# MyrtleSoftware/myrtlespeech

Measured on AMD Instinct MI355X. Metric: audio-sec/s (RTF), DS2 5xBiLSTM-1024 encoder forward + CTC greedy, 80-feature 10 s clips @ batch 32/GPU, higher is better.
Workload: dtype f16x3 (f32 split in fp16 hi+lo, 3 fp16 MFMA passes, f32 acc: LSTM, projections, conv1/2, FC1; FC2/CTC/decode f32)

## Files before the change

include/ms_hotpath.h:

```cpp
#ifndef MS_HOTPATH_H
#define MS_HOTPATH_H

#include <stddef.h>
#include <stdint.h>

#ifdef __cplusplus
extern "C" {
#endif

#define MS_ABI_VERSION 4

enum {
  MS_OK = 0,
  MS_ERR_INVALID = 1,
  MS_ERR_HIP = 2,
  MS_ERR_WORKSPACE = 3,
  MS_ERR_TIMEOUT = 4,
  MS_ERR_UNSUPPORTED = 5
};

enum { MS_CELL_LSTM = 0, MS_CELL_GRU = 1, MS_CELL_RNN_TANH = 2, MS_CELL_HARD_LSTM = 3 };

enum { MS_ACT_NONE = 0, MS_ACT_CLAMP = 1  };

int ms_abi_version(void);
const char* ms_last_error(void);


int ms_mask_time_(float* x, const int32_t* lens, int N, int inner, int T, void* stream);

size_t ms_maskconv_packed_bytes(int Cout, int Cin_g, int KF, int KT, int groups);

int ms_maskconv_pack(const float* w, void* packed, int Cout, int Cin_g, int KF, int KT, int groups, void* stream);

int ms_maskconv_forward(const float* x, const int32_t* lens, const void* packed_w, const float* bias, float* y,
                        int N, int Cin, int Fin, int Tin, int Cout, int Fout, int Tout, int KF, int KT, int SF,
                        int ST, int DF, int DT, int pad_f_l, int pad_t_l, int groups, int act, float act_lo,
                        float act_hi, void* stream);

size_t ms_maskconv_cl_packed_bytes(int Cout, int Cin, int KF, int KT);
int ms_maskconv_cl_pack(const float* w, void* packed, int Cout, int Cin, int KF, int KT, void* stream);
size_t ms_maskconv_cl_workspace_bytes(int N, int Cin, int Fin, int Tin);
int ms_maskconv_cl_forward(const float* x, const int32_t* lens, const void* packed_w, const float* bias, float* y,
                           int N, int Cin, int Fin, int Tin, int Cout, int Fout, int Tout, int KF, int KT, int SF,
                           int ST, int DF, int DT, int pad_f_l, int pad_t_l, int act, float act_lo, float act_hi,
                           void* workspace, size_t workspace_bytes, void* stream);

size_t ms_maskconv_fwin_packed_bytes(int Cout, int KF, int KT);
int ms_maskconv_fwin_pack(const float* w, void* packed, int Cout, int KF, int KT, void* stream);
size_t ms_maskconv_fwin_workspace_bytes(int N, int Tin, int KF, int SF, int Fout);
int ms_maskconv_fwin_forward(const float* x, const int32_t* lens, const void* packed_w, const float* bias, float* y, int N,
                             int Fin, int Tin, int Cout, int Fout, int Tout, int KF, int KT, int SF, int ST, int DT,
                             int pad_f_l, int pad_t_l, int act, float act_lo, float act_hi, void* workspace,
                             size_t workspace_bytes, void* stream);

size_t ms_maskconv1d_gemm_packed_bytes(int Cout, int Cin, int KT);
int ms_maskconv1d_gemm_pack(const float* w, void* packed, int Cout, int Cin, int KT, void* stream);
size_t ms_maskconv1d_gemm_workspace_bytes(int N, int Cin, int Tout, int Cout, int KT);
int ms_maskconv1d_gemm_forward(const float* x, const int32_t* lens, const void* packed, const float* bias, float* y, int N,
                               int Cin, int Tin, int Cout, int Tout, int KT, int ST, int DT, int pad_l, int act,
                               float act_lo, float act_hi, void* workspace, size_t workspace_bytes, void* stream);

int ms_nct_to_tnc(const float* x, float* y, int N, int CF, int T, void* stream);

int ms_clamp(const float* x, float* y, size_t n, float lo, float hi, void* stream);


int ms_linear_forward(const float* x, const float* w, const float* bias, float* y, int M, int K, int N, int act,
                      float act_lo, float act_hi, void* stream);

#define MS_LINEAR_FEW_ROWS 1
size_t ms_linear_splitk_workspace_bytes(int M, int K, int N, int flags);
int ms_linear_splitk_forward(const float* x, const float* w, const float* bias, float* y, int M, int K, int N, int act,
                             float act_lo, float act_hi, int flags, void* workspace, size_t workspace_bytes, void* stream);

size_t ms_linear_split_workspace_bytes(int M, int K, int N);
int ms_linear_split_forward(const float* x, const float* w, const float* bias, float* y, int M, int K, int N, int act,
                            float act_lo, float act_hi, void* workspace, size_t workspace_bytes, void* stream);

size_t ms_linear_split_packed_bytes(int K, int N);
int ms_linear_split_pack(const float* w, void* packed, int K, int N, void* stream);
int ms_linear_split_forward_packed(const float* x, const void* packed_w, const float* bias, float* y, int M, int K, int N, int act,
                                   float act_lo, float act_hi, void* workspace, size_t workspace_bytes, void* stream);


int ms_lookahead_forward(const float* x, const float* w, float* y, int N, int F, int T, int ctx, long xs_n,
                         long xs_f, long xs_t, long ys_n, long ys_f, long ys_t, int act, float act_lo,
// ... 180 lines not shown
```

myrtlespeech_amd/_lib.py:

```python
import ctypes
import os
import re
from ctypes import POINTER, c_char_p, c_double, c_float, c_int, c_int32, c_long, c_size_t, c_void_p

import torch

_HERE = os.path.dirname(os.path.abspath(__file__))
LIB_PATH = os.environ.get("MS_HOTPATH_LIB") or os.path.join(_HERE, "libms_hotpath.so")
HEADER_PATH = os.path.join(os.path.dirname(_HERE), "include", "ms_hotpath.h")

MS_OK = 0
ABI_VERSION = 4
ERR_NAMES = {1: "MS_ERR_INVALID", 2: "MS_ERR_HIP", 3: "MS_ERR_WORKSPACE", 4: "MS_ERR_TIMEOUT", 5: "MS_ERR_UNSUPPORTED"}

CELL_LSTM, CELL_GRU, CELL_RNN_TANH, CELL_HARD_LSTM = 0, 1, 2, 3
ACT_NONE, ACT_CLAMP = 0, 1
LINEAR_FEW_ROWS = 1
PROF_KINDS = 9

_P = c_void_p
_PP = POINTER(c_void_p)

SIGNATURES = {
    "ms_abi_version": (c_int, []),
    "ms_last_error": (c_char_p, []),
    "ms_mask_time_": (c_int, [_P, _P, c_int, c_int, c_int, _P]),
    "ms_maskconv_packed_bytes": (c_size_t, [c_int, c_int, c_int, c_int, c_int]),
    "ms_maskconv_pack": (c_int, [_P, _P, c_int, c_int, c_int, c_int, c_int, _P]),
    "ms_maskconv_forward": (c_int, [_P, _P, _P, _P, _P] + [c_int] * 17 + [c_float, c_float, _P]),
    "ms_maskconv_cl_packed_bytes": (c_size_t, [c_int, c_int, c_int, c_int]),
    "ms_maskconv_cl_pack": (c_int, [_P, _P, c_int, c_int, c_int, c_int, _P]),
    "ms_maskconv_cl_workspace_bytes": (c_size_t, [c_int, c_int, c_int, c_int]),
    "ms_maskconv_cl_forward": (c_int, [_P, _P, _P, _P, _P] + [c_int] * 16 + [c_float, c_float, _P, c_size_t, _P]),
    "ms_maskconv_fwin_packed_bytes": (c_size_t, [c_int, c_int, c_int]),
    "ms_maskconv_fwin_pack": (c_int, [_P, _P, c_int, c_int, c_int, _P]),
    "ms_maskconv_fwin_workspace_bytes": (c_size_t, [c_int, c_int, c_int, c_int, c_int]),
    "ms_maskconv_fwin_forward": (c_int, [_P, _P, _P, _P, _P] + [c_int] * 14 + [c_float, c_float, _P, c_size_t, _P]),
    "ms_maskconv1d_gemm_packed_bytes": (c_size_t, [c_int, c_int, c_int]),
    "ms_maskconv1d_gemm_pack": (c_int, [_P, _P, c_int, c_int, c_int, _P]),
    "ms_maskconv1d_gemm_workspace_bytes": (c_size_t, [c_int] * 5),
    "ms_maskconv1d_gemm_forward": (c_int, [_P, _P, _P, _P, _P] + [c_int] * 10 + [c_float, c_float, _P, c_size_t, _P]),
    "ms_nct_to_tnc": (c_int, [_P, _P, c_int, c_int, c_int, _P]),
    "ms_clamp": (c_int, [_P, _P, c_size_t, c_float, c_float, _P]),
    "ms_linear_forward": (c_int, [_P, _P, _P, _P, c_int, c_int, c_int, c_int, c_float, c_float, _P]),
    "ms_linear_splitk_workspace_bytes": (c_size_t, [c_int, c_int, c_int, c_int]),
    "ms_linear_splitk_forward": (c_int, [_P, _P, _P, _P, c_int, c_int, c_int, c_int, c_float, c_float, c_int, _P, c_size_t, _P]),
    "ms_linear_split_workspace_bytes": (c_size_t, [c_int, c_int, c_int]),
    "ms_linear_split_forward": (c_int, [_P, _P, _P, _P, c_int, c_int, c_int, c_int, c_float, c_float, _P, c_size_t, _P]),
    "ms_linear_split_packed_bytes": (c_size_t, [c_int, c_int]),
    "ms_linear_split_pack": (c_int, [_P, _P, c_int, c_int, _P]),
    "ms_linear_split_forward_packed": (c_int, [_P, _P, _P, _P, c_int, c_int, c_int, c_int, c_float, c_float, _P, c_size_t, _P]),
    "ms_lookahead_forward": (c_int, [_P, _P, _P, c_int, c_int, c_int, c_int] + [c_long] * 6 + [c_int, c_float, c_float, _P]),
    "ms_lookahead_window_forward": (c_int, [_P, _P, _P, c_int, c_int, c_int, c_int, c_int] + [c_long] * 6 + [c_int, c_float, c_float, _P]),
    "ms_rnn_packed_bytes": (c_size_t, [c_int, c_int, c_int, c_int]),
    "ms_ctc_status": (c_int, [_P, _P]),
    "ms_rnn_padded_hidden": (c_int, [c_int, c_int, c_int]),
    "ms_rnn_hx_preinit": (c_int, [c_int] * 8 + [_P, c_size_t, _P]),
    "ms_rnn_pack": (c_int, [c_int, c_int, c_int, c_int, _PP, _PP, _PP, _PP, _P, _P]),
    "ms_rnn_workspace_bytes": (c_size_t, [c_int] * 6),
    "ms_rnn_layer_forward": (c_int, [c_int, _P, _P, _P, c_int, _P, _P, _P, _P, _P] + [c_int] * 5 + [_P, c_size_t, _P]),
    "ms_rnn_layer_forward_ex": (c_int, [c_int, _P, _P, _P, c_int, _P, _P, _P, _P, _P] + [c_int] * 6 + [_P, c_size_t, _P]),
    "ms_rnn_layer_chains_planes": (c_int, [c_int, c_int, c_int]),
    "ms_rnn_layer_is_wide": (c_int, [c_int] * 4),
    "ms_rnn_stack_overlap_ok": (c_int, [c_int] * 7),
    "ms_rnn_stack_forward": (c_int, [c_int, _P, _P, _P, c_int, _P, _P, _P, _P, _P] + [c_int] * 7 + [_P, c_size_t, _P]),
    "ms_rnn_status": (c_int, [_P, _P]),
    "ms_rnn_debug_offset": (c_size_t, [c_int] * 6),
    "ms_rnn_layer_packs_rows": (c_int, [c_int] * 6),
    "ms_gemm_set_variant": (c_int, [c_int]),
    "ms_prof_enable": (c_int, [c_int]),
# ... 248 lines not shown
```

myrtlespeech_amd/csrc/conv_cl.hip:

```cpp
#include <algorithm>
#include <type_traits>

#include "common.h"

namespace {

typedef unsigned u32x4 __attribute__((ext_vector_type(4)));
typedef unsigned u32x2 __attribute__((ext_vector_type(2)));
typedef __bf16 bf16x8 __attribute__((ext_vector_type(8)));
typedef _Float16 f16x8 __attribute__((ext_vector_type(8)));

constexpr int CL_F = 2;

struct ClP {
  int N, Cin, Fin, Tin, Cout, Fout, Tout, KF, KT, SF, ST, DF, DT, pad_f, pad_t;
  int KG;
  int PW;
  int co_tiles;
  int act;
  float lo, hi;
  int FP;
};

__device__ __forceinline__ unsigned bf16b(float x) { return (unsigned)__builtin_bit_cast(unsigned short, (__bf16)x); }
// ... 120 lines not shown
            } else {
              const u32x4 bl = *reinterpret_cast<const u32x4*>(Pl + poff);
              acc[f] = ms::mfma_32x32x16<HM>(ah, bh, acc[f]);
              acc[f] = ms::mfma_32x32x16<HM>(al, bh, acc[f]);
              acc[f] = ms::mfma_32x32x16<HM>(ah, bl, acc[f]);
            }
          }
        }
      }
    }
    __syncthreads();
  }

  const int t = t0 + wt * 32 + l31;
  const float winv = scale_word[1];
  if (t < p.Tout) {
#pragma unroll
    for (int f = 0; f < CL_F; ++f) {
      const int fo = fo0 + wf * CL_F + f;
      if (fo >= p.Fout) continue;
#pragma unroll
      for (int r = 0; r < 16; ++r) {
        const int co = tile * 32 + ms::mfma32_row(r, lane);
        if (co < p.Cout) {
          float v = acc[f][r] * winv + (bias ? bias[co] : 0.f);
          if (p.act == MS_ACT_CLAMP) v = fminf(fmaxf(v, p.lo), p.hi);
          y[(((size_t)n * p.Cout + co) * p.Fout + fo) * p.Tout + t] = v;
        }
      }
    }
  }
}


constexpr int SH_RB = 12;
constexpr int SH_KT = 11;

template <int P>
__global__ __launch_bounds__(256, 1) void maskconv_cl_short_kernel(const unsigned short* __restrict__ xh,
                                                                   const unsigned short* __restrict__ xl,
                                                                   const int32_t* __restrict__ lens,
                                                                   const unsigned short* __restrict__ wp,
                                                                   const float* __restrict__ bias, float* __restrict__ y, ClP p,
                                                                   int RB, int RIN, const float* __restrict__ scale_word) {
  constexpr bool F16 = ms::prec_one_plane(P), HM = P == ms::PREC_F16X3;
  const float winv = scale_word[1];
  extern __shared__ __attribute__((aligned(16))) char lds[];
  const int tid = threadIdx.x, lane = tid & 63, wave = __builtin_amdgcn_readfirstlane(tid >> 6);
  const int c16 = lane & 15, q = lane >> 4;
  const int fo0 = blockIdx.x * RB, cb = blockIdx.y, n = blockIdx.z;
  const int PW = p.PW;
  const int row_bytes = PW * 64;
  char* Ph = lds;
  char* Pl = lds + (size_t)RIN * row_bytes;
  const int len = lens ? min(lens[n], p.Tin) : p.Tin;
  const int fin_lo = fo0 * p.SF - p.pad_f;

  for (int i = tid; i < RIN * PW * 4; i += 256) {
    const int kg = i & 3, rq = i >> 2;
    const int r = rq / PW, fq = rq - r * PW;
    const int fin = fin_lo + r, tin = fq - p.pad_t;
    u32x4 vh = {0u, 0u, 0u, 0u}, vl = {0u, 0u, 0u, 0u};
    if (fin >= 0 && fin < p.Fin && tin >= 0 && tin < len) {
      const size_t off = (((size_t)n * p.Fin + fin) * p.Tin + tin) * 32 + kg * 8;
      vh = *reinterpret_cast<const u32x4*>(xh + off);
      if (!F16) vl = *reinterpret_cast<const u32x4*>(xl + off);
// ... 173 lines not shown
  }
  return 0;
}

template <bool WIN>
int conv_cl_launch(const ClP& p, int wf, size_t lds, const unsigned short* xh, const unsigned short* xl, const int32_t* lens,
                   const void* packed_w, const float* bias, float* y, hipStream_t stream, const float* scale_word) {
  static ms::DeviceOnce attr_once;
  if (attr_once.need()) {
#define MS_CL_ATTR(PP)                                                                                                                     \
    MS_HIP(hipFuncSetAttribute((const void*)maskconv_cl_kernel<PP, WIN, 1>, hipFuncAttributeMaxDynamicSharedMemorySize, 160 * 1024));   \
    MS_HIP(hipFuncSetAttribute((const void*)maskconv_cl_kernel<PP, WIN, 4>, hipFuncAttributeMaxDynamicSharedMemorySize, 160 * 1024));
    MS_CL_ATTR(ms::PREC_BF16X3) MS_CL_ATTR(ms::PREC_F16) MS_CL_ATTR(ms::PREC_F16X3)
#undef MS_CL_ATTR
    attr_once.done();
  }
  const int prec = ms::split_mode();
  const int tt = 128 / wf, rf = CL_F * wf;
  dim3 grid(ms::cdiv(p.Tout, tt), ms::cdiv(p.Fout, rf), p.N * p.co_tiles);
  const unsigned short* wq = (const unsigned short*)packed_w;
#define MS_CL_LAUNCH(WF_)                                                                                                             \
  if (prec == ms::PREC_F16) hipLaunchKernelGGL((maskconv_cl_kernel<ms::PREC_F16, WIN, WF_>), grid, dim3(256), lds, stream, xh, xl, lens, wq, bias, y, p, scale_word); \
  else if (prec == ms::PREC_F16X3) hipLaunchKernelGGL((maskconv_cl_kernel<ms::PREC_F16X3, WIN, WF_>), grid, dim3(256), lds, stream, xh, xl, lens, wq, bias, y, p, scale_word); \
  else hipLaunchKernelGGL((maskconv_cl_kernel<ms::PREC_BF16X3, WIN, WF_>), grid, dim3(256), lds, stream, xh, xl, lens, wq, bias, y, p, scale_word);
  if (wf == 4) { MS_CL_LAUNCH(4) } else { MS_CL_LAUNCH(1) }
#undef MS_CL_LAUNCH
  MS_LAUNCH_CHECK();
  return MS_OK;
}

inline int fwin_kfp(int KF) { return ms::cdiv(KF, 16) * 16; }
inline int fwin_fp(int KF, int SF, int Fout) { return ms::cdiv((Fout - 1) * SF + fwin_kfp(KF), 32) * 32; }

}

static size_t fwin_plane_bytes(int Cout, int KF, int KT) {
  return ms::align_up((size_t)2 * KT * (fwin_kfp(KF) / 8) * (ms::cdiv(Cout, 32) * 32) * 8 * sizeof(unsigned short), 256);
}
extern "C" size_t ms_maskconv_fwin_packed_bytes(int Cout, int KF, int KT) {
  if (Cout <= 0 || KF <= 0 || KT <= 0) return 0;
  return fwin_plane_bytes(Cout, KF, KT) + 256;
}

extern "C" int ms_maskconv_fwin_pack(const float* w, void* packed, int Cout, int KF, int KT, void* stream) {
  MS_REQUIRE(w && packed, "null pointer");
  MS_REQUIRE(Cout > 0 && KF > 0 && KT > 0, "bad shape");
  const int cout_pad = ms::cdiv(Cout, 32) * 32, KG = fwin_kfp(KF) / 8;
  const size_t plane = (size_t)KT * KG * cout_pad * 8;
  const int blocks = (int)std::min<size_t>((plane + 255) / 256, 2048);
  float* scale_word = (float*)((char*)packed + fwin_plane_bytes(Cout, KF, KT));
  const int rc = ms::weight_scale_launch(w, (size_t)Cout * KF * KT, scale_word, ms::split_mode(), (hipStream_t)stream);
  if (rc != MS_OK) return rc;
  hipLaunchKernelGGL(conv_fwin_pack_kernel, dim3(blocks), dim3(256), 0, (hipStream_t)stream, w, (unsigned short*)packed, Cout,
                     KF, KT, KG, cout_pad, ms::split_mode(), scale_word);
  MS_LAUNCH_CHECK();
  return MS_OK;
}

extern "C" size_t ms_maskconv_fwin_workspace_bytes(int N, int Tin, int KF, int SF, int Fout) {
  if (N <= 0 || Tin <= 0 || KF <= 0 || SF <= 0 || Fout <= 0) return 0;
  return ms::align_up((size_t)N * Tin * fwin_fp(KF, SF, Fout) * 4, 256);
}

extern "C" int ms_maskconv_fwin_forward(const float* x, const int32_t* lens, const void* packed_w, const float* bias, float* y,
                                        int N, int Fin, int Tin, int Cout, int Fout, int Tout, int KF, int KT, int SF, int ST,
                                        int DT, int pad_f_l, int pad_t_l, int act, float act_lo, float act_hi, void* workspace,
                                        size_t workspace_bytes, void* stream_) {
  ms::ProfScope prof_span(MS_PROF_CONV, (hipStream_t)stream_);
  MS_REQUIRE(x && packed_w && y && workspace, "null pointer");
  MS_REQUIRE(N > 0 && Fin > 0 && Tin > 0 && Cout > 0 && Fout > 0 && Tout > 0, "bad shape");
  MS_REQUIRE(KF > 0 && KT > 0 && SF > 0 && ST > 0 && DT > 0 && pad_f_l >= 0 && pad_t_l >= 0, "bad kernel");
  MS_REQUIRE(SF % 2 == 0, "feature stride must be even (4-byte aligned window loads)");
  MS_REQUIRE(act == MS_ACT_NONE || act == MS_ACT_CLAMP, "bad act");
  if (workspace_bytes < ms_maskconv_fwin_workspace_bytes(N, Tin, KF, SF, Fout)) {
    ms::set_error("ms_maskconv_fwin_forward: workspace too small");
    return MS_ERR_WORKSPACE;
  }
  hipStream_t stream = (hipStream_t)stream_;
  ClP p;
  p.N = N; p.Cin = fwin_kfp(KF); p.Fin = 1; p.Tin = Tin; p.Cout = Cout; p.Fout = Fout; p.Tout = Tout; p.KF = 1; p.KT = KT;
  p.SF = SF; p.ST = ST; p.DF = 1; p.DT = DT; p.pad_f = 0; p.pad_t = pad_t_l; p.KG = p.Cin / 8;
  p.co_tiles = ms::cdiv(Cout, 32);
  p.act = act; p.lo = act_lo; p.hi = act_hi;
  p.FP = fwin_fp(KF, SF, Fout);
  size_t lds = 0;
  const int wf = conv_cl_plan(p, &lds);
  if (wf == 0 || (size_t)N * Tin * p.FP * 2 >= ((size_t)1 << 31)) {
    ms::set_error("ms_maskconv_fwin_forward: shape outside the LDS / grid budget");
    return MS_ERR_UNSUPPORTED;
  }
  unsigned short* xh = (unsigned short*)workspace;
  unsigned short* xl = xh + (size_t)N * Tin * p.FP;
  const int prec = ms::split_mode();
  const bool f16 = prec == ms::PREC_F16;
  hipLaunchKernelGGL(ft_to_tf_split_kernel, dim3(ms::cdiv(Tin, 32), ms::cdiv(p.FP, 32), N), dim3(32, 8), 0, stream, x, xh, xl,
                     Fin, Tin, p.FP, pad_f_l, prec);
  MS_LAUNCH_CHECK();
  return conv_cl_launch<true>(p, wf, lds, xh, xl, lens, packed_w, bias, y, stream,
                              (const float*)((const char*)packed_w + fwin_plane_bytes(Cout, KF, KT)));
}

static size_t cl_plane_bytes(int Cout, int Cin, int KF, int KT) {
  return ms::align_up((size_t)2 * KF * KT * (Cin / 8) * (ms::cdiv(Cout, 32) * 32) * 8 * sizeof(unsigned short), 256);
}
extern "C" size_t ms_maskconv_cl_packed_bytes(int Cout, int Cin, int KF, int KT) {
  if (Cout <= 0 || Cin <= 0 || Cin % 16 || KF <= 0 || KT <= 0) return 0;
  return cl_plane_bytes(Cout, Cin, KF, KT) + 256;
}

extern "C" int ms_maskconv_cl_pack(const float* w, void* packed, int Cout, int Cin, int KF, int KT, void* stream) {
  MS_REQUIRE(w && packed, "null pointer");
  MS_REQUIRE(Cout > 0 && Cin > 0 && Cin % 16 == 0 && KF > 0 && KT > 0, "bad shape (Cin must be a multiple of 16)");
  const int cout_pad = ms::cdiv(Cout, 32) * 32;
  const size_t plane = (size_t)KF * KT * (Cin / 8) * cout_pad * 8;
  const int blocks = (int)std::min<size_t>((plane + 255) / 256, 2048);
  float* scale_word = (float*)((char*)packed + cl_plane_bytes(Cout, Cin, KF, KT));
  const int rc = ms::weight_scale_launch(w, (size_t)Cout * Cin * KF * KT, scale_word, ms::split_mode(), (hipStream_t)stream);
  if (rc != MS_OK) return rc;
  hipLaunchKernelGGL(conv_cl_pack_kernel, dim3(blocks), dim3(256), 0, (hipStream_t)stream, w, (unsigned short*)packed, Cout,
                     Cin, KF, KT, cout_pad, ms::split_mode(), scale_word);
  MS_LAUNCH_CHECK();
  return MS_OK;
}

extern "C" size_t ms_maskconv_cl_workspace_bytes(int N, int Cin, int Fin, int Tin) {
  if (N <= 0 || Cin <= 0 || Fin <= 0 || Tin <= 0) return 0;
  return ms::align_up((size_t)N * Cin * Fin * Tin * 4, 256);
}

extern "C" int ms_maskconv_cl_forward(const float* x, const int32_t* lens, const void* packed_w, const float* bias, float* y,
                                      int N, int Cin, int Fin, int Tin, int Cout, int Fout, int Tout, int KF, int KT,
                                      int SF, int ST, int DF, int DT, int pad_f_l, int pad_t_l, int act, float act_lo,
                                      float act_hi, void* workspace, size_t workspace_bytes, void* stream_) {
  ms::ProfScope prof_span(MS_PROF_CONV, (hipStream_t)stream_);
  MS_REQUIRE(x && packed_w && y && workspace, "null pointer");
  MS_REQUIRE(N > 0 && Cin > 0 && Cin % 16 == 0 && Fin > 0 && Tin > 0 && Cout > 0 && Fout > 0 && Tout > 0, "bad shape");
  MS_REQUIRE(KF > 0 && KT > 0 && SF > 0 && ST > 0 && DF > 0 && DT > 0 && pad_f_l >= 0 && pad_t_l >= 0, "bad kernel");
  MS_REQUIRE(act == MS_ACT_NONE || act == MS_ACT_CLAMP, "bad act");
  if (workspace_bytes < ms_maskconv_cl_workspace_bytes(N, Cin, Fin, Tin)) {
    ms::set_error("ms_maskconv_cl_forward: workspace too small");
    return MS_ERR_WORKSPACE;
  }
  hipStream_t stream = (hipStream_t)stream_;
  ClP p;
  p.N = N; p.Cin = Cin; p.Fin = Fin; p.Tin = Tin; p.Cout = Cout; p.Fout = Fout; p.Tout = Tout; p.KF = KF; p.KT = KT;
  p.SF = SF; p.ST = ST; p.DF = DF; p.DT = DT; p.pad_f = pad_f_l; p.pad_t = pad_t_l; p.KG = Cin / 8;
  p.co_tiles = ms::cdiv(Cout, 32);
  p.act = act; p.lo = act_lo; p.hi = act_hi;
  p.FP = 0;
  size_t lds = 0;
  const int wf = conv_cl_plan(p, &lds);
  if (wf == 0) {
    ms::set_error("ms_maskconv_cl_forward: shape outside the LDS / grid budget");
    return MS_ERR_UNSUPPORTED;
  }
  const float* scale_word = (const float*)((const char*)packed_w + cl_plane_bytes(Cout, Cin, KF, KT));
  unsigned short* xh = (unsigned short*)workspace;
  unsigned short* xl = xh + (size_t)N * Cin * Fin * Tin;
  MS_REQUIRE(N * Fin <= 65535, "N*Fin exceeds grid limits");
  const int prec = ms::split_mode();
  const bool f16 = prec == ms::PREC_F16;
  hipLaunchKernelGGL(nchw_to_cl_split_kernel, dim3(ms::cdiv(Tin, 32), ms::cdiv(Cin, 32), N * Fin), dim3(32, 8), 0, stream, x,
                     xh, xl, Cin, Fin, Tin, prec);
  MS_LAUNCH_CHECK();
  {
    int RB = 0, RIN = 0;
    size_t slds = 0;
    if (conv_cl_short_plan(p, f16, &RB, &RIN, &slds)) {
      static ms::DeviceOnce attr_once;
      if (attr_once.need()) {
        MS_HIP(hipFuncSetAttribute((const void*)maskconv_cl_short_kernel<ms::PREC_BF16X3>, hipFuncAttributeMaxDynamicSharedMemorySize, 160 * 1024));
        MS_HIP(hipFuncSetAttribute((const void*)maskconv_cl_short_kernel<ms::PREC_F16>, hipFuncAttributeMaxDynamicSharedMemorySize, 160 * 1024));
        MS_HIP(hipFuncSetAttribute((const void*)maskconv_cl_short_kernel<ms::PREC_F16X3>, hipFuncAttributeMaxDynamicSharedMemorySize, 160 * 1024));
        attr_once.done();
      }
      ClP ps = p;
      ps.PW = Tout + KT - 1;
      const dim3 grid(ms::cdiv(Fout, RB), ms::cdiv(Cout, 16), N);
      const unsigned short* wq = (const unsigned short*)packed_w;
      auto kern = prec == ms::PREC_F16 ? maskconv_cl_short_kernel<ms::PREC_F16>
                  : prec == ms::PREC_F16X3 ? maskconv_cl_short_kernel<ms::PREC_F16X3> : maskconv_cl_short_kernel<ms::PREC_BF16X3>;
      hipLaunchKernelGGL(kern, grid, dim3(256), slds, stream, xh, xl, lens, wq, bias, y, ps, RB, RIN, scale_word);
      MS_LAUNCH_CHECK();
      return MS_OK;
    }
  }
  return conv_cl_launch<false>(p, wf, lds, xh, xl, lens, packed_w, bias, y, stream, scale_word);
}
```

myrtlespeech_amd/model/cnn.py:

```python
from enum import Enum
import os
from typing import List, Optional, Tuple, TypeVar, Union

import torch

from myrtlespeech_amd import _lib


class PaddingMode(Enum):

    NONE = 0
    SAME = 1


def pad_same(length: int, kernel_size: int, stride: int = 1, dilation: int = 1) -> Tuple[int, int]:
    for name, v in (("length", length), ("kernel_size", kernel_size), ("stride", stride), ("dilation", dilation)):
        if v <= 0:
            raise ValueError(f"{name}={v} must be > 0")
    span = dilation * (kernel_size - 1) + 1
    n_out = (length + stride - 1) // stride
    total = stride * n_out - 1 + span - length
    left = total // 2
    return left, total - left

# ... 74 lines not shown
    n, cin, fin, tin = x4.shape
    cout, _, kf, kt = weight4.shape
    (sf, st), (df, dt) = stride, dilation
    if same:
        pt = pad_same(tin, kt, st, dt)
        pf = pad_same(fin, kf, sf, df)
    else:
        pt = pf = (0, 0)
    if time_pads is not None:
        pt = (int(time_pads[0]), int(time_pads[1]))
    fout = (fin + sum(pf) - (df * (kf - 1) + 1)) // sf + 1
    tout = (tin + sum(pt) - (dt * (kt - 1) + 1)) // st + 1
    if fout <= 0 or tout <= 0:
        raise RuntimeError("convolution output would be empty")
    host_in = _lib.host_lens(seq_lens).to(seq_lens.dtype)
    new_host = out_lens(host_in, kt, st, dt, sum(pt))
    new_lens = _lib.attach_host(_lib.upload(new_host), new_host)
    y = torch.empty((n, cout, fout, tout), dtype=torch.float32, device="cuda")
    lens_dev = _lib.lens_i32(seq_lens)
    a, lo, hi = (_lib.ACT_NONE, 0.0, 0.0) if act is None else (_lib.ACT_CLAMP, act[0], act[1])
    b = None if bias is None else _lib.f32c(bias.detach())
    big = 2.0 * y.numel() * cin * kf * kt >= float(os.environ.get("MS_CONV_MFMA_MIN_FLOPS", "1e9"))
    if _lib.split_precision() and groups == 1 and fin == 1 and kf == 1 and sf == 1 and pf == (0, 0) and cin * kt >= 64 and big:
        pk = packed.get_gemm1d(weight4)
        nbytes = lib.ms_maskconv1d_gemm_workspace_bytes(n, cin, tout, cout, kt)
        ws = packed.workspace.get(nbytes)
        _lib.check(lib.ms_maskconv1d_gemm_forward(_lib.ptr(x4), _lib.ptr(lens_dev), _lib.ptr(pk), _lib.ptr(b), _lib.ptr(y), n,
                                                  cin, tin, cout, tout, kt, st, dt, pt[0], a, lo, hi, _lib.ptr(ws), nbytes,
                                                  _lib.stream_ptr()), "ms_maskconv1d_gemm_forward")
        return y, new_lens
    if _lib.split_precision() and groups == 1 and cin % 16 == 0 and big:
        pk = packed.get_cl(weight4)
        ws = packed.workspace.get(lib.ms_maskconv_cl_workspace_bytes(n, cin, fin, tin))
        rc = lib.ms_maskconv_cl_forward(_lib.ptr(x4), _lib.ptr(lens_dev), _lib.ptr(pk), _lib.ptr(b), _lib.ptr(y), n, cin,
                                        fin, tin, cout, fout, tout, kf, kt, sf, st, df, dt, pf[0], pt[0], a, lo, hi,
                                        _lib.ptr(ws), ws.numel(), _lib.stream_ptr())
        if rc != 5:
            _lib.check(rc, "ms_maskconv_cl_forward")
            return y, new_lens
    big_fwin = 2.0 * y.numel() * cin * kf * kt >= float(os.environ.get("MS_CONV_MFMA_MIN_FLOPS", "2e8"))
    if (_lib.split_precision() and groups == 1 and cin == 1 and df == 1 and sf % 2 == 0 and kf >= 16 and big_fwin
            and os.environ.get("MS_CONV_FWIN") != "0"):
        pk = packed.get_fwin(weight4)
        nbytes = lib.ms_maskconv_fwin_workspace_bytes(n, tin, kf, sf, fout)
        ws = packed.workspace.get(nbytes)
        rc = lib.ms_maskconv_fwin_forward(_lib.ptr(x4), _lib.ptr(lens_dev), _lib.ptr(pk), _lib.ptr(b), _lib.ptr(y), n, fin,
                                          tin, cout, fout, tout, kf, kt, sf, st, dt, pf[0], pt[0], a, lo, hi, _lib.ptr(ws),
                                          nbytes, _lib.stream_ptr())
        if rc != 5:
            _lib.check(rc, "ms_maskconv_fwin_forward")
            return y, new_lens
    pk = packed.get(weight4, groups)
    _lib.check(lib.ms_maskconv_forward(_lib.ptr(x4), _lib.ptr(lens_dev), _lib.ptr(pk), _lib.ptr(b), _lib.ptr(y), n, cin,
                                       fin, tin, cout, fout, tout, kf, kt, sf, st, df, dt, pf[0], pt[0], groups, a, lo,
                                       hi, _lib.stream_ptr()), "ms_maskconv_forward")
    return y, new_lens


def _mask_in_place(acts: torch.Tensor, seq_lens: torch.Tensor):
    if acts.is_cuda and acts.dtype == torch.float32 and acts.is_contiguous():
        n, t = acts.shape[0], acts.shape[-1]
        h = _lib.host_lens(seq_lens)
        if h.numel() == n and n and int(h.min()) >= t:
            return True
        inner = acts.numel() // (n * t)
        lens_dev = _lib.lens_i32(seq_lens)
        _lib.check(_lib.load().ms_mask_time_(_lib.ptr(acts), _lib.ptr(lens_dev), n, inner, t, _lib.stream_ptr()),
                   "ms_mask_time_")
        return True
    return False


class MaskConv1d(torch.nn.Conv1d):

    def __init__(self, in_channels: int, out_channels: int, kernel_size: int, stride: int = 1,
                 padding_mode: PaddingMode = PaddingMode.NONE, dilation: int = 1, groups: int = 1, bias: bool = True):
        super().__init__(in_channels=in_channels, out_channels=out_channels, kernel_size=kernel_size, stride=stride,
                         dilation=dilation, groups=groups, bias=bias)
        if padding_mode not in (PaddingMode.NONE, PaddingMode.SAME):
            raise ValueError(f"unknown padding mode {padding_mode}")
        self._padding_mode = padding_mode
# ... 83 lines not shown
```

Before: 26910.

## Add specialized pipelined MFMA conv kernel for KT=11 channel-last and fwin convs

Adds a fixed-shape conv kernel specialized for the DS2 conv shapes (KT=11, KG=4 or 6). It stages input rows and weight taps in LDS with register prefetch of the next kf slice or tap group, double-buffers operand reads, and interleaves MFMA with LDS reads using scheduling barriers. Both the conv1 fwin path and the conv2 channel-last path try this kernel first and fall back to the generic one when the shape does not match. It adds code specialized to these exact shapes. The large LDS footprint may also limit occupancy.

```diff
diff --git a/include/ms_hotpath.h b/include/ms_hotpath.h
--- a/include/ms_hotpath.h
+++ b/include/ms_hotpath.h
@@ -53,6 +53,16 @@
                              int Fin, int Tin, int Cout, int Fout, int Tout, int KF, int KT, int SF, int ST, int DT,
                              int pad_f_l, int pad_t_l, int act, float act_lo, float act_hi, void* workspace,
                              size_t workspace_bytes, void* stream);
+
+int ms_maskconv_cl_fast_supported(int Cin, int KF, int KT, int ST, int DT, int Tout, int fwin);
+int ms_maskconv_cl_fast_forward(const float* x, const int32_t* lens, const void* packed_w, const float* bias, float* y,
+                                int N, int Cin, int Fin, int Tin, int Cout, int Fout, int Tout, int KF, int KT, int SF,
+                                int ST, int DF, int DT, int pad_f_l, int pad_t_l, int act, float act_lo, float act_hi,
+                                void* workspace, size_t workspace_bytes, void* stream);
+int ms_maskconv_fwin_fast_forward(const float* x, const int32_t* lens, const void* packed_w, const float* bias, float* y,
+                                  int N, int Fin, int Tin, int Cout, int Fout, int Tout, int KF, int KT, int SF, int ST,
+                                  int DT, int pad_f_l, int pad_t_l, int act, float act_lo, float act_hi, void* workspace,
+                                  size_t workspace_bytes, void* stream);
 
 size_t ms_maskconv1d_gemm_packed_bytes(int Cout, int Cin, int KT);
 int ms_maskconv1d_gemm_pack(const float* w, void* packed, int Cout, int Cin, int KT, void* stream);
diff --git a/myrtlespeech_amd/_lib.py b/myrtlespeech_amd/_lib.py
--- a/myrtlespeech_amd/_lib.py
+++ b/myrtlespeech_amd/_lib.py
@@ -36,6 +36,9 @@
     "ms_maskconv_fwin_pack": (c_int, [_P, _P, c_int, c_int, c_int, _P]),
     "ms_maskconv_fwin_workspace_bytes": (c_size_t, [c_int, c_int, c_int, c_int, c_int]),
     "ms_maskconv_fwin_forward": (c_int, [_P, _P, _P, _P, _P] + [c_int] * 14 + [c_float, c_float, _P, c_size_t, _P]),
+    "ms_maskconv_cl_fast_supported": (c_int, [c_int] * 7),
+    "ms_maskconv_cl_fast_forward": (c_int, [_P, _P, _P, _P, _P] + [c_int] * 16 + [c_float, c_float, _P, c_size_t, _P]),
+    "ms_maskconv_fwin_fast_forward": (c_int, [_P, _P, _P, _P, _P] + [c_int] * 14 + [c_float, c_float, _P, c_size_t, _P]),
     "ms_maskconv1d_gemm_packed_bytes": (c_size_t, [c_int, c_int, c_int]),
     "ms_maskconv1d_gemm_pack": (c_int, [_P, _P, c_int, c_int, c_int, _P]),
     "ms_maskconv1d_gemm_workspace_bytes": (c_size_t, [c_int] * 5),
diff --git a/myrtlespeech_amd/csrc/conv_cl.hip b/myrtlespeech_amd/csrc/conv_cl.hip
--- a/myrtlespeech_amd/csrc/conv_cl.hip
+++ b/myrtlespeech_amd/csrc/conv_cl.hip
@@ -176,6 +176,223 @@
   }
 }
 
+template <bool WIN>
+struct ClFast {
+  static constexpr int KG = WIN ? 6 : 4, KT = 11, ST = WIN ? 2 : 1;
+  static constexpr int PW = 127 * ST + KT;
+  static constexpr int HW = (PW + 1) / 2;
+  static constexpr int PWS = WIN ? 2 * HW : PW;
+  static constexpr int NGRAN = KG * PW;
+  static constexpr int ROW_BYTES = KG * PWS * 16;
+  static constexpr int NT0 = WIN ? 6 : KT;
+  static constexpr int W_BYTES = NT0 * KG * 32 * 16;
+  static constexpr int LDS_BYTES = 2 * CL_F * ROW_BYTES + 2 * W_BYTES;
+  static constexpr int NIT_X = (CL_F * NGRAN + 255) / 256;
+  static constexpr int NIT_W = (NT0 * KG * 32 + 255) / 256;
+};
+
+template <int P, bool WIN>
+__global__ __launch_bounds__(256, WIN ? 1 : 2) void maskconv_cl_fast_kernel(const unsigned short* __restrict__ xh,
+                                                                            const unsigned short* __restrict__ xl,
+                                                                            const int32_t* __restrict__ lens,
+                                                                            const unsigned short* __restrict__ wp,
+                                                                            const float* __restrict__ bias,
+                                                                            float* __restrict__ y, ClP p,
+                                                                            const float* __restrict__ scale_word) {
+  using S = ClFast<WIN>;
+  constexpr bool HM = P == ms::PREC_F16X3;
+  constexpr int KG = S::KG, KT = S::KT;
+  extern __shared__ __attribute__((aligned(16))) char lds[];
+  char* Ph = lds;
+  char* Pl = lds + CL_F * S::ROW_BYTES;
+  char* Wh = lds + 2 * CL_F * S::ROW_BYTES;
+  char* Wl = Wh + S::W_BYTES;
+
+  const int tid = threadIdx.x, lane = tid & 63, wt = tid >> 6;
+  const int l31 = lane & 31, half = lane >> 5;
+  const int t0 = blockIdx.x * 128;
+  const int fo0 = blockIdx.y * CL_F;
+  const int n = blockIdx.z / p.co_tiles, tile = blockIdx.z % p.co_tiles;
+  const int len = lens ? min(lens[n], p.Tin) : p.Tin;
+  const int cout_pad = p.co_tiles * 32;
+  const size_t wplane = (size_t)p.KF * KT * KG * cout_pad * 8;
+  const int tin0 = t0 * S::ST - p.pad_t;
+  const unsigned plane_bytes = WIN ? (unsigned)((size_t)p.N * p.Tin * p.FP * 2) : 0u;
+  const __amdgpu_buffer_rsrc_t xh_rsrc = __builtin_amdgcn_make_buffer_rsrc(const_cast<unsigned short*>(xh), 0, plane_bytes, 0x00020000);
+  const __amdgpu_buffer_rsrc_t xl_rsrc = __builtin_amdgcn_make_buffer_rsrc(const_cast<unsigned short*>(xl), 0, plane_bytes, 0x00020000);
+
+  ms::f32x16 acc[CL_F];
+#pragma unroll
+  for (int f = 0; f < CL_F; ++f)
+#pragma unroll
+    for (int r = 0; r < 16; ++r) acc[f][r] = 0.f;
+
+  u32x4 xrh[S::NIT_X], xrl[S::NIT_X], wrh[S::NIT_W], wrl[S::NIT_W];
+
+  auto load_rows = [&](int kf) {
+#pragma unroll
+    for (int it = 0; it < S::NIT_X; ++it) {
+      const int i = tid + it * 256;
+      const int f = i / S::NGRAN, r = i - f * S::NGRAN;
+      const int q = r / KG, kg = r - q * KG;
+      const int fo = fo0 + f, tin = tin0 + q;
+      const int fin = fo * p.SF - p.pad_f + kf * p.DF;
+      const bool ok = i < CL_F * S::NGRAN && fo < p.Fout && tin >= 0 && tin < len && (WIN || (fin >= 0 && fin < p.Fin));
+      u32x4 vh = {0u, 0u, 0u, 0u}, vl = {0u, 0u, 0u, 0u};
+      if (ok) {
+        if (WIN) {
+          const int boff = (int)((((size_t)n * p.Tin + tin) * p.FP + (size_t)fo * p.SF + kg * 8) * 2);
+          vh = __builtin_amdgcn_raw_buffer_load_b128(xh_rsrc, boff, 0, 0);
+          vl = __builtin_amdgcn_raw_buffer_load_b128(xl_rsrc, boff, 0, 0);
+        } else {
+          const size_t off = (((size_t)n * p.Fin + fin) * p.Tin + tin) * (KG * 8) + kg * 8;
+          vh = *reinterpret_cast<const u32x4*>(xh + off);
+          vl = *reinterpret_cast<const u32x4*>(xl + off);
+        }
+      }
+      xrh[it] = vh;
+      xrl[it] = vl;
+    }
+  };
+  auto store_rows = [&]() {
+#pragma unroll
+    for (int it = 0; it < S::NIT_X; ++it) {
+      const int i = tid + it * 256;
+      const int f = i / S::NGRAN, r = i - f * S::NGRAN;
+      const int q = r / KG, kg = r - q * KG;
+      const int slot = WIN ? (q & 1) * S::HW + (q >> 1) : q;
+      if (i < CL_F * S::NGRAN) {
+        const int off = f * S::ROW_BYTES + (kg * S::PWS + slot) * 16;
+        *reinterpret_cast<u32x4*>(Ph + off) = xrh[it];
+        *reinterpret_cast<u32x4*>(Pl + off) = xrl[it];
+      }
+    }
+  };
+  auto load_taps = [&](int kf, auto kt0_, auto nt_) {
+    constexpr int kt0 = decltype(kt0_)::value, nt = decltype(nt_)::value;
+#pragma unroll
+    for (int it = 0; it < S::NIT_W; ++it) {
+      const int i = tid + it * 256;
+      if (i < nt * KG * 32) {
+        const int co = i & 31, rest = i >> 5;
+        const size_t src = ((((size_t)kf * KT + kt0) * KG + rest) * cout_pad + tile * 32 + co) * 8;
+        wrh[it] = *reinterpret_cast<const u32x4*>(wp + src);
+        wrl[it] = *reinterpret_cast<const u32x4*>(wp + wplane + src);
+      }
+    }
+  };
+  auto store_taps = [&](auto nt_) {
+    constexpr int nt = decltype(nt_)::value;
+#pragma unroll
+    for (int it = 0; it < S::NIT_W; ++it) {
+      const int i = tid + it * 256;
+      if (i < nt * KG * 32) {
+        *reinterpret_cast<u32x4*>(Wh + i * 16) = wrh[it];
+        *reinterpret_cast<u32x4*>(Wl + i * 16) = wrl[it];
+      }
+    }
+  };
+  const int a_lane = (half * 32 + l31) * 16;
+  const int b_lane = (half * S::PWS + wt * 32 + l31) * 16;
+  auto compute = [&](auto kt0_, auto nt_) {
+    constexpr int kt0 = decltype(kt0_)::value, nt = decltype(nt_)::value;
+    constexpr int NS = nt * (KG / 2);
+    u32x4 ah[2], al[2], bh[2][CL_F], bl[2][CL_F];
+    auto read = [&](int set, int step) {
+      const int ktl = step / (KG / 2), s = step - ktl * (KG / 2);
+      const int kt = kt0 + ktl;
+      const int slot = WIN ? (kt & 1) * S::HW + (kt >> 1) : kt;
+      const int woff = a_lane + (ktl * KG + 2 * s) * 32 * 16;
+      ah[set] = *reinterpret_cast<const u32x4*>(Wh + woff);
+      al[set] = *reinterpret_cast<const u32x4*>(Wl + woff);
+#pragma unroll
+      for (int f = 0; f < CL_F; ++f) {
+        const int poff = b_lane + f * S::ROW_BYTES + (2 * s * S::PWS + slot) * 16;
+        bh[set][f] = *reinterpret_cast<const u32x4*>(Ph + poff);
+        bl[set][f] = *reinterpret_cast<const u32x4*>(Pl + poff);
+      }
+    };
+    read(0, 0);
+    __builtin_amdgcn_sched_barrier(0);
+#pragma unroll
+    for (int step = 0; step < NS; ++step) {
+      const int c = step & 1;
+      if (step + 1 < NS) read(c ^ 1, step + 1);
+#pragma unroll
+      for (int f = 0; f < CL_F; ++f) acc[f] = ms::mfma_32x32x16<HM>(ah[c], bh[c][f], acc[f]);
+#pragma unroll
+      for (int f = 0; f < CL_F; ++f) acc[f] = ms::mfma_32x32x16<HM>(al[c], bh[c][f], acc[f]);
+#pragma unroll
+      for (int f = 0; f < CL_F; ++f) acc[f] = ms::mfma_32x32x16<HM>(ah[c], bl[c][f], acc[f]);
+      if (step + 1 < NS) {
+#pragma unroll
+        for (int i = 0; i < 3 * CL_F; ++i) {
+          __builtin_amdgcn_sched_group_barrier(0x008, 1, 0);
+          __builtin_amdgcn_sched_group_barrier(0x100, 1, 0);
+        }
+      }
+      __builtin_amdgcn_sched_barrier(0);
+    }
+  };
+
+  constexpr std::integral_constant<int, 0> T0{};
+  constexpr std::integral_constant<int, S::NT0> NA{};
+  load_rows(0);
+  load_taps(0, T0, NA);
+  store_rows();
+  store_taps(NA);
+  __syncthreads();
+  if constexpr (WIN) {
+    constexpr std::integral_constant<int, KT - S::NT0> NB{};
+    load_taps(0, NA, NB);
+    compute(T0, NA);
+    __syncthreads();
+    store_taps(NB);
+    __syncthreads();
+    compute(NA, NB);
+  } else {
+    for (int kf = 0; kf < p.KF; ++kf) {
+      const bool more = kf + 1 < p.KF;
+      if (more) {
+        load_rows(kf + 1);
+        load_taps(kf + 1, T0, NA);
+      }
+      compute(T0, NA);
+      if (more) {
+        __syncthreads();
+        store_rows();
+        store_taps(NA);
+        __syncthreads();
+      }
+    }
+  }
+
+  const int t = t0 + wt * 32 + l31;
+  const float winv = scale_word[1];
+  float bv[16];
+#pragma unroll
+  for (int r = 0; r < 16; ++r) {
+    const int co = tile * 32 + ms::mfma32_row(r, lane);
+    bv[r] = (bias && co < p.Cout) ? bias[co] : 0.f;
+  }
+  if (t < p.Tout) {
+#pragma unroll
+    for (int f = 0; f < CL_F; ++f) {
+      const int fo = fo0 + f;
+      if (fo >= p.Fout) continue;
+#pragma unroll
+      for (int r = 0; r < 16; ++r) {
+        const int co = tile * 32 + ms::mfma32_row(r, lane);
+        if (co < p.Cout) {
+          float v = acc[f][r] * winv + bv[r];
+          if (p.act == MS_ACT_CLAMP) v = fminf(fmaxf(v, p.lo), p.hi);
+          y[(((size_t)n * p.Cout + co) * p.Fout + fo) * p.Tout + t] = v;
+        }
+      }
+    }
+  }
+}
+
 
 constexpr int SH_RB = 12;
 constexpr int SH_KT = 11;
@@ -415,6 +632,44 @@
 inline int fwin_kfp(int KF) { return ms::cdiv(KF, 16) * 16; }
 inline int fwin_fp(int KF, int SF, int Fout) { return ms::cdiv((Fout - 1) * SF + fwin_kfp(KF), 32) * 32; }
 
+template <bool WIN>
+int conv_cl_fast_launch(const ClP& p, const unsigned short* xh, const unsigned short* xl, const int32_t* lens,
+                        const void* packed_w, const float* bias, float* y, hipStream_t stream, const float* scale_word) {
+  using S = ClFast<WIN>;
+  static_assert(S::LDS_BYTES <= (WIN ? 160 : 80) * 1024, "LDS budget");
+  static ms::DeviceOnce attr_once;
+  if (attr_once.need()) {
+    MS_HIP(hipFuncSetAttribute((const void*)maskconv_cl_fast_kernel<ms::PREC_BF16X3, WIN>, hipFuncAttributeMaxDynamicSharedMemorySize, 160 * 1024));
+    MS_HIP(hipFuncSetAttribute((const void*)maskconv_cl_fast_kernel<ms::PREC_F16X3, WIN>, hipFuncAttributeMaxDynamicSharedMemorySize, 160 * 1024));
+    attr_once.done();
+  }
+  const dim3 grid(ms::cdiv(p.Tout, 128), ms::cdiv(p.Fout, CL_F), p.N * p.co_tiles);
+  const unsigned short* wq = (const unsigned short*)packed_w;
+  static const bool alone = getenv("MS_CONV_CL_FAST_ALONE") && getenv("MS_CONV_CL_FAST_ALONE")[0] == '1';
+  const size_t lds = alone ? std::max<size_t>(S::LDS_BYTES, 96 * 1024) : S::LDS_BYTES;
+  if (ms::split_mode() == ms::PREC_F16X3)
+    hipLaunchKernelGGL((maskconv_cl_fast_kernel<ms::PREC_F16X3, WIN>), grid, dim3(256), lds, stream, xh, xl, lens, wq, bias, y, p, scale_word);
+  else
+    hipLaunchKernelGGL((maskconv_cl_fast_kernel<ms::PREC_BF16X3, WIN>), grid, dim3(256), lds, stream, xh, xl, lens, wq, bias, y, p, scale_word);
+  MS_LAUNCH_CHECK();
+  return MS_OK;
+}
+template <bool WIN>
+bool conv_cl_fast_shape(int KG, int KT, int ST, int DT, int Tout) {
+  return KG == ClFast<WIN>::KG && KT == ClFast<WIN>::KT && ST == ClFast<WIN>::ST && DT == 1 && Tout > 48;
+}
+template <bool WIN>
+bool conv_cl_fast_ok(const ClP& p) {
+  return conv_cl_fast_shape<WIN>(p.KG, p.KT, p.ST, p.DT, p.Tout) && ms::split_mode() != ms::PREC_F16 &&
+         (long)p.N * p.co_tiles <= 65535 && ms::cdiv(p.Fout, CL_F) <= 65535;
+}
+
+}
+
+extern "C" int ms_maskconv_cl_fast_supported(int Cin, int KF, int KT, int ST, int DT, int Tout, int fwin) {
+  if (Cin <= 0 || KF <= 0) return 0;
+  if (fwin) return Cin == 1 && conv_cl_fast_shape<true>(fwin_kfp(KF) / 8, KT, ST, DT, Tout);
+  return Cin % 16 == 0 && conv_cl_fast_shape<false>(Cin / 8, KT, ST, DT, Tout);
 }
 
 static size_t fwin_plane_bytes(int Cout, int KF, int KT) {
@@ -445,10 +700,10 @@
   return ms::align_up((size_t)N * Tin * fwin_fp(KF, SF, Fout) * 4, 256);
 }
 
-extern "C" int ms_maskconv_fwin_forward(const float* x, const int32_t* lens, const void* packed_w, const float* bias, float* y,
-                                        int N, int Fin, int Tin, int Cout, int Fout, int Tout, int KF, int KT, int SF, int ST,
-                                        int DT, int pad_f_l, int pad_t_l, int act, float act_lo, float act_hi, void* workspace,
-                                        size_t workspace_bytes, void* stream_) {
+static int ms_maskconv_fwin_forward_impl(bool fast, const float* x, const int32_t* lens, const void* packed_w, const float* bias, float* y,
+                        int N, int Fin, int Tin, int Cout, int Fout, int Tout, int KF, int KT, int SF, int ST,
+                        int DT, int pad_f_l, int pad_t_l, int act, float act_lo, float act_hi, void* workspace,
+                        size_t workspace_bytes, void* stream_) {
   ms::ProfScope prof_span(MS_PROF_CONV, (hipStream_t)stream_);
   MS_REQUIRE(x && packed_w && y && workspace, "null pointer");
   MS_REQUIRE(N > 0 && Fin > 0 && Tin > 0 && Cout > 0 && Fout > 0 && Tout > 0, "bad shape");
@@ -472,6 +727,10 @@
     ms::set_error("ms_maskconv_fwin_forward: shape outside the LDS / grid budget");
     return MS_ERR_UNSUPPORTED;
   }
+  if (fast && !conv_cl_fast_ok<true>(p)) {
+    ms::set_error("ms_maskconv_fwin_fast_forward: not a shape of the pipelined kernel");
+    return MS_ERR_UNSUPPORTED;
+  }
   unsigned short* xh = (unsigned short*)workspace;
   unsigned short* xl = xh + (size_t)N * Tin * p.FP;
   const int prec = ms::split_mode();
@@ -479,8 +738,23 @@
   hipLaunchKernelGGL(ft_to_tf_split_kernel, dim3(ms::cdiv(Tin, 32), ms::cdiv(p.FP, 32), N), dim3(32, 8), 0, stream, x, xh, xl,
                      Fin, Tin, p.FP, pad_f_l, prec);
   MS_LAUNCH_CHECK();
-  return conv_cl_launch<true>(p, wf, lds, xh, xl, lens, packed_w, bias, y, stream,
-                              (const float*)((const char*)packed_w + fwin_plane_bytes(Cout, KF, KT)));
+  const float* scale_word = (const float*)((const char*)packed_w + fwin_plane_bytes(Cout, KF, KT));
+  if (fast) return conv_cl_fast_launch<true>(p, xh, xl, lens, packed_w, bias, y, stream, scale_word);
+  return conv_cl_launch<true>(p, wf, lds, xh, xl, lens, packed_w, bias, y, stream, scale_word);
+}
+extern "C" int ms_maskconv_fwin_forward(const float* x, const int32_t* lens, const void* packed_w, const float* bias, float* y,
+                                        int N, int Fin, int Tin, int Cout, int Fout, int Tout, int KF, int KT, int SF, int ST,
+                                        int DT, int pad_f_l, int pad_t_l, int act, float act_lo, float act_hi, void* workspace,
+                                        size_t workspace_bytes, void* stream_) {
+  return ms_maskconv_fwin_forward_impl(false, x, lens, packed_w, bias, y, N, Fin, Tin, Cout, Fout, Tout, KF, KT, SF, ST, DT, pad_f_l, pad_t_l,
+                      act, act_lo, act_hi, workspace, workspace_bytes, stream_);
+}
+extern "C" int ms_maskconv_fwin_fast_forward(const float* x, const int32_t* lens, const void* packed_w, const float* bias,
+                                             float* y, int N, int Fin, int Tin, int Cout, int Fout, int Tout, int KF, int KT,
+                                             int SF, int ST, int DT, int pad_f_l, int pad_t_l, int act, float act_lo,
+                                             float act_hi, void* workspace, size_t workspace_bytes, void* stream_) {
+  return ms_maskconv_fwin_forward_impl(true, x, lens, packed_w, bias, y, N, Fin, Tin, Cout, Fout, Tout, KF, KT, SF, ST, DT, pad_f_l, pad_t_l,
+                      act, act_lo, act_hi, workspace, workspace_bytes, stream_);
 }
 
 static size_t cl_plane_bytes(int Cout, int Cin, int KF, int KT) {
@@ -511,10 +785,10 @@
   return ms::align_up((size_t)N * Cin * Fin * Tin * 4, 256);
 }
 
-extern "C" int ms_maskconv_cl_forward(const float* x, const int32_t* lens, const void* packed_w, const float* bias, float* y,
-                                      int N, int Cin, int Fin, int Tin, int Cout, int Fout, int Tout, int KF, int KT,
-                                      int SF, int ST, int DF, int DT, int pad_f_l, int pad_t_l, int act, float act_lo,
-                                      float act_hi, void* workspace, size_t workspace_bytes, void* stream_) {
+static int ms_maskconv_cl_forward_impl(bool fast, const float* x, const int32_t* lens, const void* packed_w, const float* bias, float* y,
+                      int N, int Cin, int Fin, int Tin, int Cout, int Fout, int Tout, int KF, int KT,
+                      int SF, int ST, int DF, int DT, int pad_f_l, int pad_t_l, int act, float act_lo,
+                      float act_hi, void* workspace, size_t workspace_bytes, void* stream_) {
   ms::ProfScope prof_span(MS_PROF_CONV, (hipStream_t)stream_);
   MS_REQUIRE(x && packed_w && y && workspace, "null pointer");
   MS_REQUIRE(N > 0 && Cin > 0 && Cin % 16 == 0 && Fin > 0 && Tin > 0 && Cout > 0 && Fout > 0 && Tout > 0, "bad shape");
@@ -537,6 +811,10 @@
     ms::set_error("ms_maskconv_cl_forward: shape outside the LDS / grid budget");
     return MS_ERR_UNSUPPORTED;
   }
+  if (fast && !conv_cl_fast_ok<false>(p)) {
+    ms::set_error("ms_maskconv_cl_fast_forward: not a shape of the pipelined kernel");
+    return MS_ERR_UNSUPPORTED;
+  }
   const float* scale_word = (const float*)((const char*)packed_w + cl_plane_bytes(Cout, Cin, KF, KT));
   unsigned short* xh = (unsigned short*)workspace;
   unsigned short* xl = xh + (size_t)N * Cin * Fin * Tin;
@@ -546,6 +824,7 @@
   hipLaunchKernelGGL(nchw_to_cl_split_kernel, dim3(ms::cdiv(Tin, 32), ms::cdiv(Cin, 32), N * Fin), dim3(32, 8), 0, stream, x,
                      xh, xl, Cin, Fin, Tin, prec);
   MS_LAUNCH_CHECK();
+  if (fast) return conv_cl_fast_launch<false>(p, xh, xl, lens, packed_w, bias, y, stream, scale_word);
   {
     int RB = 0, RIN = 0;
     size_t slds = 0;
@@ -570,3 +849,17 @@
   }
   return conv_cl_launch<false>(p, wf, lds, xh, xl, lens, packed_w, bias, y, stream, scale_word);
 }
+extern "C" int ms_maskconv_cl_forward(const float* x, const int32_t* lens, const void* packed_w, const float* bias, float* y,
+                                      int N, int Cin, int Fin, int Tin, int Cout, int Fout, int Tout, int KF, int KT,
+                                      int SF, int ST, int DF, int DT, int pad_f_l, int pad_t_l, int act, float act_lo,
+                                      float act_hi, void* workspace, size_t workspace_bytes, void* stream_) {
+  return ms_maskconv_cl_forward_impl(false, x, lens, packed_w, bias, y, N, Cin, Fin, Tin, Cout, Fout, Tout, KF, KT, SF, ST, DF, DT, pad_f_l,
+                    pad_t_l, act, act_lo, act_hi, workspace, workspace_bytes, stream_);
+}
+extern "C" int ms_maskconv_cl_fast_forward(const float* x, const int32_t* lens, const void* packed_w, const float* bias,
+                                           float* y, int N, int Cin, int Fin, int Tin, int Cout, int Fout, int Tout, int KF,
+                                           int KT, int SF, int ST, int DF, int DT, int pad_f_l, int pad_t_l, int act,
+                                           float act_lo, float act_hi, void* workspace, size_t workspace_bytes, void* stream_) {
+  return ms_maskconv_cl_forward_impl(true, x, lens, packed_w, bias, y, N, Cin, Fin, Tin, Cout, Fout, Tout, KF, KT, SF, ST, DF, DT, pad_f_l,
+                    pad_t_l, act, act_lo, act_hi, workspace, workspace_bytes, stream_);
+}
diff --git a/myrtlespeech_amd/model/cnn.py b/myrtlespeech_amd/model/cnn.py
--- a/myrtlespeech_amd/model/cnn.py
+++ b/myrtlespeech_amd/model/cnn.py
@@ -130,9 +130,13 @@
     if _lib.split_precision() and groups == 1 and cin % 16 == 0 and big:
         pk = packed.get_cl(weight4)
         ws = packed.workspace.get(lib.ms_maskconv_cl_workspace_bytes(n, cin, fin, tin))
-        rc = lib.ms_maskconv_cl_forward(_lib.ptr(x4), _lib.ptr(lens_dev), _lib.ptr(pk), _lib.ptr(b), _lib.ptr(y), n, cin,
-                                        fin, tin, cout, fout, tout, kf, kt, sf, st, df, dt, pf[0], pt[0], a, lo, hi,
-                                        _lib.ptr(ws), ws.numel(), _lib.stream_ptr())
+        args = (_lib.ptr(x4), _lib.ptr(lens_dev), _lib.ptr(pk), _lib.ptr(b), _lib.ptr(y), n, cin, fin, tin, cout, fout, tout,
+                kf, kt, sf, st, df, dt, pf[0], pt[0], a, lo, hi, _lib.ptr(ws), ws.numel(), _lib.stream_ptr())
+        rc = 5
+        if os.environ.get("MS_CONV_CL_FAST") != "0" and lib.ms_maskconv_cl_fast_supported(cin, kf, kt, st, dt, tout, 0):
+            rc = lib.ms_maskconv_cl_fast_forward(*args)
+        if rc == 5:
+            rc = lib.ms_maskconv_cl_forward(*args)
         if rc != 5:
             _lib.check(rc, "ms_maskconv_cl_forward")
             return y, new_lens
@@ -142,9 +146,13 @@
         pk = packed.get_fwin(weight4)
         nbytes = lib.ms_maskconv_fwin_workspace_bytes(n, tin, kf, sf, fout)
         ws = packed.workspace.get(nbytes)
-        rc = lib.ms_maskconv_fwin_forward(_lib.ptr(x4), _lib.ptr(lens_dev), _lib.ptr(pk), _lib.ptr(b), _lib.ptr(y), n, fin,
-                                          tin, cout, fout, tout, kf, kt, sf, st, dt, pf[0], pt[0], a, lo, hi, _lib.ptr(ws),
-                                          nbytes, _lib.stream_ptr())
+        args = (_lib.ptr(x4), _lib.ptr(lens_dev), _lib.ptr(pk), _lib.ptr(b), _lib.ptr(y), n, fin, tin, cout, fout, tout, kf,
+                kt, sf, st, dt, pf[0], pt[0], a, lo, hi, _lib.ptr(ws), nbytes, _lib.stream_ptr())
+        rc = 5
+        if os.environ.get("MS_CONV_CL_FAST") != "0" and lib.ms_maskconv_cl_fast_supported(1, kf, kt, st, dt, tout, 1):
+            rc = lib.ms_maskconv_fwin_fast_forward(*args)
+        if rc == 5:
+            rc = lib.ms_maskconv_fwin_forward(*args)
         if rc != 5:
             _lib.check(rc, "ms_maskconv_fwin_forward")
             return y, new_lens
```

Result: faster. 27420, median of 6 (+1.9%).
